# sgartkink/opencl-spmv-algorithms

Measured on AMD Instinct MI355X. Metric: effective HBM GB/s + GFLOP/s per format on cant.mtx, 1/2/4/8 MI355X, higher is better.
Workload: dtype f64

## Files before the change

### include/spmv_ext.h

```cpp
#ifndef SPMV_EXT_H
#define SPMV_EXT_H

#include "spmv.h"

#ifdef __cplusplus
extern "C" {
#endif

size_t spmv_coo_tail_bytes(int64_t nnz);
int spmv_coo_tail_build(spmv_dims d, const int32_t *row, void *tails, size_t tails_bytes);
int spmv_coo_run_tail(spmv_dims d, const int32_t *row, const int32_t *col, const double *val,
                      const double *x, double *y, const void *tails);

int spmv_csr_run_variant(spmv_dims d, const int64_t *row_ptr,
                         const int32_t *col, const double *val,
                         const double *x, double *y, int lanes_per_row,
                         int variant);
size_t spmv_csr_xwin_bytes(int64_t n_rows, int64_t nnz, int lanes_per_row, int32_t rows_per_window);
int spmv_csr_xwin_build(spmv_dims d, const int64_t *row_ptr, const int32_t *col, int lanes_per_row,
                        int32_t rows_per_window, void *win, size_t win_bytes, int32_t *xcap);
int spmv_csr_run_xwin(spmv_dims d, const int64_t *row_ptr, const int32_t *col, const double *val,
                      const double *x, double *y, int lanes_per_row, int32_t rows_per_window,
                      const void *win, int32_t xcap);
int spmv_csr16_run(spmv_dims d, const int64_t *row_ptr, const int32_t *blk_base,
// ... 132 lines not shown

int spmv_dev_csr_from_coo(spmv_dims d, const int32_t *row, const int32_t *col, const double *val,
                          int64_t *row_ptr, int32_t *col_out, double *val_out);
int spmv_dev_ell_plan(spmv_dims d, const int64_t *row_ptr, int32_t ki, int32_t *K, int64_t *ld);
int spmv_dev_ell_fill(spmv_dims d, const int64_t *row_ptr, const int32_t *col, const double *val,
                      int32_t K, int64_t ld, int32_t ki, int32_t *col_out, double *val_out);
int spmv_dev_sell_plan(spmv_dims d, const int64_t *row_ptr, const int32_t *col, int32_t C,
                       int32_t sigma, int32_t ki, int64_t n_slices, int32_t *perm, int64_t *slice_ptr,
                       int32_t *slice_col, int64_t *stored);
int spmv_dev_sell_fill(spmv_dims d, const int64_t *row_ptr, const int32_t *col, const double *val,
                       int32_t C, int32_t ki, int64_t n_slices, const int64_t *slice_ptr,
                       const int32_t *perm, const int32_t *slice_col, int32_t *col_out,
                       double *val_out);
int spmv_dev_cmrs_build(spmv_dims d, const int64_t *row_ptr, int32_t h, int64_t *strip_ptr,
                        uint8_t *row_in_strip);
int spmv_dev_csr_transpose(spmv_dims d, const int64_t *row_ptr, const int32_t *col, const double *val,
                           int64_t *t_ptr, int32_t *t_col, double *t_val);

size_t spmv_dot_ws_bytes(int64_t n);
int spmv_dot(int64_t n, const double *a, const double *b, double *out, void *ws,
             size_t ws_bytes, int device, void *stream);
int spmv_axpy_ratio(int64_t n, const double *num, const double *den, double sign,
                    const double *x, double *y, int device, void *stream);
int spmv_xpay_ratio(int64_t n, const double *num, const double *den, const double *x,
                    double *y, int device, void *stream);
int spmv_scale_rsqrt(int64_t n, const double *s, const double *x, double *y, int device,
                     void *stream);
int spmv_gather(int64_t n, const int32_t *order, const double *x, double *out, int device, void *stream);

enum spmv_option {
    SPMV_OPT_XWIN_REMAP = 1,
    SPMV_OPT_XCD_REMAP = 2,
    SPMV_OPT_STREAM_NT = 3,
    SPMV_OPT_CSR_PREFETCH = 4
};
int spmv_set_option(int option, int value);
int spmv_get_option(int option);


#ifdef __cplusplus
}
#endif

#endif
```

### opencl-spmv-algorithms_amd/csrc/common.h

```cpp
#pragma once

#include <hip/hip_runtime.h>
#include <stdint.h>

#include <type_traits>

#include "spmv.h"
#include "spmv_ext.h"

namespace spmv {

constexpr int kWave = 64;
constexpr int kBlock = 256;

int fail(int rc, const char *where, hipError_t e);
int fail_msg(int rc, const char *msg);

template <int V0, int... Vs, typename F>
inline auto with_int(int v, F &&f)
{
    if constexpr (sizeof...(Vs) == 0)
        return f(std::integral_constant<int, V0>{});
    else if (v == V0)
        return f(std::integral_constant<int, V0>{});
    else
        return with_int<Vs...>(v, f);
}

template <typename F>
inline auto with_bool(bool b, F &&f)
{
    if (b)
        return f(std::true_type{});
    else
        return f(std::false_type{});
}

class DeviceGuard {
  public:
    explicit DeviceGuard(int dev);
    ~DeviceGuard();
    int rc() const { return rc_; }

  private:
    int prev_ = -1;
    int rc_ = SPMV_SUCCESS;
};

bool xcd_remap_enabled();
bool xwin_remap(bool dflt);
bool csr_prefetch(bool dflt);
bool sell_small(int32_t C, int64_t n_slices);

int launch_cmrs_staged(const spmv_dims &d, int32_t h, int64_t n_strips,
                       const int64_t *strip_ptr, const uint8_t *rin, const int32_t *col,
                       const double *val, const double *x, double *y, const int2 *win = nullptr,
                       int32_t xcap = 0);
void cmrs_geometry(const spmv_dims &d, int32_t h, int64_t n_strips, int *L, int *G, int64_t *blocks);
int launch_coo_staged(const spmv_dims &d, const int32_t *row, const int32_t *col,
                      const double *val, const double *x, double *y, int32_t *carry_row,
                      double *carry_val, const int2 *win = nullptr, int32_t xcap = 0,
                      const int32_t *tails = nullptr);
int64_t coo_tail_build(const spmv_dims &d, const int32_t *row, int32_t *tails);
int64_t coo_tail_cap();
int windows_download(const void *win, int64_t n, hipStream_t st, int2 **host, const char *who);
int windows_xcap(const void *win, int64_t n, int32_t cap, hipStream_t st, int32_t *xcap, const char *who);
constexpr int32_t kStagedXwinCap = 2048;
int64_t coo_staged_tile();
int64_t coo_hot_tile(int64_t n_rows, int64_t nnz);
int launch_coo_staged_acc(const spmv_dims &d, const int32_t *row, const int32_t *col,
                          const double *val, const double *x, double *y, int32_t *carry_row,
                          double *carry_val, const int32_t *tails = nullptr);
int launch_csr_tiled(const spmv_dims &d, const int64_t *row_ptr, const int32_t *col,
                     const double *val, const double *x, double *y, int32_t *own_lo,
                     int32_t *carry_row, double *carry_val);
int64_t csr_tiled_tile(int64_t n_rows, int64_t nnz);
int64_t csr_tiled_tile_min();
template <typename V>
int launch_csr_tiled_hot(const spmv_dims &d, const int64_t *row_ptr, const int32_t *col,
                         const V *val, const double *x, double *y, int64_t H, const int32_t *hot,
                         double *xh, const int32_t *own_lo_plan, int32_t *own_lo, int32_t *carry_row,
                         double *carry_val, const int32_t *big = nullptr, int64_t big_len = 0);
int launch_cmrs_tiled(const spmv_dims &d, int32_t h, int64_t n_strips, const int64_t *strip_ptr,
                      const uint8_t *rin, const int32_t *col, const double *val, const double *x,
                      double *y, int32_t *own_lo, int32_t *carry_row, double *carry_val, int64_t H = 0,
                      const int32_t *hot = nullptr, double *xh = nullptr, bool own_lo_ready = false);
int cmrs_tiled_planned(const spmv_dims &d, int32_t h, int64_t n_strips, const int64_t *strip_ptr,
                       const uint8_t *rin, const int32_t *col, const double *val, const double *x, double *y,
                       int64_t H, const int32_t *hot, void *ws, bool fill);
__global__ void csr_tile_rows_kernel(int64_t n_rows, int64_t nnz, int64_t tiles, int64_t ch,
                                     const int64_t *__restrict__ ptr, int32_t *__restrict__ own_lo);
struct XHot;
int launch_coo_staged_acc_hot(const spmv_dims &d, const int32_t *row, const int32_t *col,
                              const double *val, const double *x, double *y, int32_t *carry_row,
                              double *carry_val, const XHot xs);
int launch_coo_staged_hot(const spmv_dims &d, const int32_t *row, const int32_t *col, const double *val,
                          const double *x, double *y, int32_t *carry_row, double *carry_val, int64_t H,
                          const int32_t *hot, double *xh);
int64_t cmrs_tiled_tile(int64_t n_rows, int64_t nnz);
// ... 244 lines not shown
```

### opencl-spmv-algorithms_amd/csrc/csr.hip

```cpp
#include <stdio.h>
#include <stdlib.h>

#include <type_traits>

#include "common.h"

namespace spmv {

template <int L, typename XS>
__device__ __forceinline__ double row_dot_pairs(int64_t beg, int64_t end, int lane,
                                                const int32_t *__restrict__ col,
                                                const double *__restrict__ val, const XS &xs)
{
    double s0 = 0.0, s1 = 0.0, s2 = 0.0, s3 = 0.0;
    int64_t p = (beg & ~(int64_t)1) + 2 * lane;
    for (; p + 1 + 2 * L < end; p += 4 * L) {
        const double2 va = *reinterpret_cast<const double2 *>(val + p);
        const int2 ca = *reinterpret_cast<const int2 *>(col + p);
        const double2 vb = *reinterpret_cast<const double2 *>(val + p + 2 * L);
        const int2 cb = *reinterpret_cast<const int2 *>(col + p + 2 * L);
        s0 += (p >= beg ? va.x : 0.0) * xs(ca.x);
        s1 += va.y * xs(ca.y);
        s2 += vb.x * xs(cb.x);
        s3 += vb.y * xs(cb.y);
// ... 14 lines not shown
template <int L>
__global__ __launch_bounds__(kBlock) void csr_vector_kernel(
    int64_t n_rows, const int64_t *__restrict__ row_ptr,
    const int32_t *__restrict__ col, const double *__restrict__ val,
    const double *__restrict__ x, double *__restrict__ y, int remap)
{
    constexpr int RPB = kBlock / L;
    __shared__ int64_t s_ptr[RPB + 1];

    const int64_t row0 = xcd_block(remap) * RPB;
    if (threadIdx.x <= RPB) {
        int64_t r = row0 + threadIdx.x;
        s_ptr[threadIdx.x] = row_ptr[r < n_rows ? r : n_rows];
    }
    __syncthreads();

    const int g = threadIdx.x / L;
    const int lane = threadIdx.x % L;
    const int64_t row = row0 + g;
    const int64_t beg = s_ptr[g], end = s_ptr[g + 1];
    const double sum = row_dot_pairs<L>(beg, end, lane, col, val, XGlobal{x});
    if (lane == 0 && row < n_rows)
        store_y(y + (row), sum);
}

constexpr int kStageRoundsDefault = 3;
constexpr int64_t kChunkAlign = 32;
__host__ __device__ __forceinline__ int64_t chunk_start(int64_t e) { return e & ~(kChunkAlign - 1); }
constexpr bool kCsrStreamNtDefault = false;
constexpr bool kCsrXwinNtDefault = true;

template <bool NT>
struct Col32 {
    const int32_t *__restrict__ col;
    using Raw = int2;
    __device__ __forceinline__ int2 pair(int64_t p) const { return stream_load2<NT>(col + p); }
    __device__ __forceinline__ int32_t one(int64_t p) const { return stream_load<NT>(col + p); }
    __device__ __forceinline__ Raw raw(int64_t p) const { return stream_load2<NT>(col + p); }
    __device__ __forceinline__ int2 decode(Raw r, int64_t) const { return r; }
};

template <bool NT>
struct Col16 {
    const int32_t *__restrict__ base;
    const uint16_t *__restrict__ off;
    const int32_t *__restrict__ esc;
    __device__ __forceinline__ int2 pair(int64_t p) const
    {
        const int32_t b = base[p >> 6];
        if (b >= 0) {
            const uint32_t w = stream_load<NT>(reinterpret_cast<const uint32_t *>(off + p));
            return int2{b + (int32_t)(w & 0xffffu), b + (int32_t)(w >> 16)};
        }
        return stream_load2<NT>(esc + (int64_t)(-1 - b) * 64 + (p & 63));
    }
    __device__ __forceinline__ int32_t one(int64_t p) const
    {
        const int32_t b = base[p >> 6];
        return b >= 0 ? b + (int32_t)stream_load<NT>(off + p) : esc[(int64_t)(-1 - b) * 64 + (p & 63)];
    }
    struct Raw {
        int32_t b;
        uint32_t w;
    };
    __device__ __forceinline__ Raw raw(int64_t p) const
    {
        return Raw{base[p >> 6], stream_load<NT>(reinterpret_cast<const uint32_t *>(off + p))};
    }
    __device__ __forceinline__ int2 decode(Raw r, int64_t p) const
    {
        if (r.b >= 0)
            return int2{r.b + (int32_t)(r.w & 0xffffu), r.b + (int32_t)(r.w >> 16)};
        return stream_load2<NT>(esc + (int64_t)(-1 - r.b) * 64 + (p & 63));
    }
};

template <int L, int R, bool NT, typename Cols = Col32<NT>, typename XS = XGlobal, typename V = double>
__device__ __forceinline__ void staged_group(
    int64_t row, const int64_t *s_ptr, double2 *s_prod,
    const Cols cols, const V *__restrict__ val,
    const XS xs, double *__restrict__ y, int64_t n_rows)
{
    constexpr int RPB = kBlock / L;
    constexpr int CH = 2 * kBlock * R;
    const int g = threadIdx.x / L;
    const int lane = threadIdx.x % L;
    const int64_t beg = s_ptr[g], end = s_ptr[g + 1];
    const int64_t blk_end = s_ptr[RPB];
    const double *prod = reinterpret_cast<const double *>(s_prod);

    double acc = 0.0;
    for (int64_t cb = chunk_start(s_ptr[0]); cb < blk_end; cb += CH) {
        const int64_t ce = cb + CH < blk_end ? cb + CH : blk_end;
#pragma unroll
        for (int k = 0; k < R; ++k) {
            const int t = threadIdx.x + k * kBlock;
            const int64_t p = cb + 2 * (int64_t)t;
            double2 pr = {0.0, 0.0};
            if (p + 1 < ce) {
                const double2 v = vpair<NT>(val + p);
                const int2 c = cols.pair(p);
                pr.x = v.x * xs(c.x);
                pr.y = v.y * xs(c.y);
            } else if (p < ce) {
                pr.x = vone<NT>(val + p) * xs(cols.one(p));
            }
// ... 172 lines not shown
    }
    for (; grp < n_groups; grp += gridDim.x) {
        if (threadIdx.x <= RPB)
            s_ptr[threadIdx.x] = next;
        __syncthreads();
        const int64_t g2 = grp + gridDim.x;
        if (threadIdx.x <= RPB && g2 < n_groups) {
            int64_t r = g2 * RPB + threadIdx.x;
            next = row_ptr[r < n_rows ? r : n_rows];
        }
        staged_group<L, R, NT, Cols>(grp * RPB + threadIdx.x / L, s_ptr, s_prod, cols, val, XGlobal{x}, y, n_rows);
    }
}

__global__ __launch_bounds__(kBlock) void csr_window_kernel(int64_t n_rows, int64_t rpb,
                                                            const int64_t *__restrict__ row_ptr,
                                                            const int32_t *__restrict__ col,
                                                            int2 *__restrict__ win)
{
    const int64_t g = blockIdx.x;
    const int64_t r1 = (g + 1) * rpb < n_rows ? (g + 1) * rpb : n_rows;
    const int64_t nz = row_ptr[n_rows];
    const int64_t b = row_ptr[g * rpb], e = row_ptr[r1];
    int2 r = {0, -1};
    if (b < e) {
        const int64_t lo = chunk_start(b) >= 2 ? chunk_start(b) - 2 : 0;
        const int64_t hi = e + 1 < nz ? e + 1 : nz;
        r = block_col_range(col, lo, hi);
    }
    if (threadIdx.x == 0)
        win[g] = r;
}

template <int L, int R, bool NT, typename V, int MODE, typename Cols>
__global__ __launch_bounds__(kBlock) void csr_xwin_kernel(
    int64_t n_rows, int64_t n_groups, int64_t gpw, const int64_t *__restrict__ row_ptr,
    const Cols cols, const V *__restrict__ val,
    const double *__restrict__ x, double *__restrict__ y, const int2 *__restrict__ win, int32_t xcap,
    int remap)
{
    static_assert(MODE == 0 || MODE == 3 || MODE == 4, "csr_xwin_kernel: MODE 0, 3 or 4");
    CSR_STAMP(0);
    constexpr int RPB = kBlock / L;
    extern __shared__ double s_x[];
    __shared__ int64_t s_ptr[MODE >= 3 ? 1 : RPB + 1];
    __shared__ double2 s_prod[kBlock * R];
    int64_t *s_off = reinterpret_cast<int64_t *>(s_x + xcap);
    const int64_t nz = row_ptr[n_rows];
    const int64_t wi = xcd_block(remap);
    const int64_t g_beg = wi * gpw;
    const int64_t g_end = (wi + 1) * gpw < n_groups ? (wi + 1) * gpw : n_groups;
    int64_t pb = 0, pe = 0, b0 = 0;
    if constexpr (MODE == 4) {
        const int64_t r0p = g_beg * RPB;
        const int64_t r1 = r0p + RPB < n_rows ? r0p + RPB : n_rows;
        b0 = row_ptr[r0p];
        pe = row_ptr[r1];
    }
    const int2 wnd = win[wi];
    if constexpr (MODE == 4) {
        asm volatile("" ::"s"(b0), "s"(pe), "s"(wnd.x), "s"(wnd.y), "s"(nz));
        pb = chunk_start(b0);
    }
    const int32_t span = wnd.y - wnd.x + 1;
    const bool staged = span > 0 && span <= xcap;
    if constexpr (MODE >= 3) {
// ... 26 lines not shown
                const int32_t i = (int32_t)threadIdx.x + k * kBlock;
                if (i < nr)
                    s_off[i] = o[k];
            }
            if (staged) {
#pragma unroll
                for (int k = 0; k < XU; ++k) {
                    const int32_t i = (int32_t)threadIdx.x + k * kBlock;
                    if (i < span)
                        s_x[i] = xv[k];
                }
            }
        } else {
        pre = false;
        for (int32_t b = 0; b < nr; b += U * kBlock) {
            int64_t o[U];
#pragma unroll
            for (int k = 0; k < U; ++k) {
                const int64_t r = r0 + b + threadIdx.x + k * kBlock;
                o[k] = row_ptr[r < n_rows ? r : n_rows];
            }
            if (staged && b == 0)
                copy_window(s_x, x, wnd.x, span);
#pragma unroll
            for (int k = 0; k < U; ++k) {
                const int32_t i = b + (int32_t)threadIdx.x + k * kBlock;
                if (i < nr)
                    s_off[i] = o[k];
            }
        }
        }
        __syncthreads();
        CSR_STAMP(1);
        if (staged)
            staged_window_pipelined<L, R, NT, XWindow, V, Cols>(r0, (int)(g_end - g_beg), s_off, s_prod, cols, val,
                                                               XWindow{s_x, wnd.x}, y, n_rows, nz, st, pre);
        else
            staged_window_pipelined<L, R, NT, XGlobal, V, Cols>(r0, (int)(g_end - g_beg), s_off, s_prod, cols, val,
                                                               XGlobal{x}, y, n_rows, nz, st, pre);
        return;
    }
    if (staged)
        for (int32_t i = threadIdx.x; i < span; i += kBlock)
            s_x[i] = x[wnd.x + i];
    for (int64_t grp = g_beg; grp < g_end; ++grp) {
        if (threadIdx.x <= RPB) {
            const int64_t r = grp * RPB + threadIdx.x;
            s_ptr[threadIdx.x] = row_ptr[r < n_rows ? r : n_rows];
        }
        __syncthreads();
        const int64_t row = grp * RPB + threadIdx.x / L;
        if (staged)
            staged_group<L, R, NT, Cols, XWindow, V>(row, s_ptr, s_prod, cols, val, XWindow{s_x, wnd.x}, y, n_rows);
        else
            staged_group<L, R, NT, Cols, XGlobal, V>(row, s_ptr, s_prod, cols, val, XGlobal{x}, y, n_rows);
    }
}

static int csr_stage_rounds(int64_t n_rows, int64_t nnz, int L)
{
    if (n_rows <= 0 || L <= 0)
        return kStageRoundsDefault;
    const double eg = (double)(kBlock / L) * ((double)nnz / (double)n_rows);
    const int64_t c3 = (int64_t)((eg + 1535.0) / 1536.0), c4 = (int64_t)((eg + 2047.0) / 2048.0);
    return c4 < c3 ? 4 : 3;
}

static int cu_count()
{
    int dev = 0, n = 0;
    if (hipGetDevice(&dev) != hipSuccess ||
        hipDeviceGetAttribute(&n, hipDeviceAttributeMultiprocessorCount, dev) != hipSuccess || n <= 0)
        n = 256;
    return n;
}

template <typename K>
static int64_t persistent_grid(K kernel, int64_t groups, size_t dyn_lds = 0)
{
    int per_cu = 0;
    if (hipOccupancyMaxActiveBlocksPerMultiprocessor(&per_cu, kernel, kBlock, dyn_lds) != hipSuccess ||
        per_cu <= 0)
        per_cu = 1;
    if (per_cu > 8)
        per_cu = 8;
// ... 158 lines not shown
static void launch_csr_xwin(const spmv_dims &d, const int64_t *row_ptr, const Cols cols,
                            const V *val, const double *x, double *y, const int2 *win, int32_t xcap,
                            int64_t gpw)
{
    constexpr int RPB = kBlock / L;
    const int64_t groups = (d.n_rows + RPB - 1) / RPB;
    const int64_t n_win = (groups + gpw - 1) / gpw;
    int mode = csr_xwin_mode(d.n_rows, d.nnz, gpw * RPB, R);
    if (mode == 3 && csr_xwin_lds(mode, xcap, gpw, RPB) + sizeof(double2) * kBlock * R * 2 > 64 * 1024)
        mode = 0;
    const size_t lds = csr_xwin_lds(mode, xcap, gpw, RPB);
    const int remap = csr_xwin_remap_rule(xcap, gpw * RPB, n_win) ? 1 : 0;
    const hipStream_t st = (hipStream_t)d.stream;
    if (mode == 3 && d.nnz >= 2 && csr_xwin_prefetch_rule(n_win))
        mode = 4;
    with_int<4, 3, 0>(mode, [&](auto M) {
        hipLaunchKernelGGL((csr_xwin_kernel<L, R, NT, V, decltype(M)::value, Cols>), dim3((unsigned)n_win),
                           dim3(kBlock), lds, st, d.n_rows, groups, gpw, row_ptr, cols, val, x, y, win, xcap, remap);
    });
}

struct MakeCol32 {
    const int32_t *col;
    template <bool NT>
    Col32<NT> get() const { return Col32<NT>{col}; }
};

struct MakeCol16 {
    const int32_t *base;
    const uint16_t *off;
    const int32_t *esc;
    template <bool NT>
    Col16<NT> get() const { return Col16<NT>{base, off, esc}; }
};

template <typename V, typename MakeCols>
static int launch_xwin_any(const spmv_dims &d, int L, const int64_t *row_ptr, MakeCols mk, const V *val,
                           const double *x, double *y, const int2 *w, int32_t xcap, int64_t gpw)
{
    if (!lanes_ok(L))
        return fail_msg(SPMV_OTHER_ERROR, "csr x-window run: lanes_per_row must be 0 or a power of two in [2,64]");
    const bool nt = stream_nt(kCsrXwinNtDefault);
    with_int<2, 4, 8, 16, 32, 64>(L, [&](auto Lc) {
        with_int<4, 3>(csr_stage_rounds(d.n_rows, d.nnz, decltype(Lc)::value), [&](auto Rc) {
            with_bool(nt, [&](auto NT) {
                launch_csr_xwin<decltype(Lc)::value, decltype(Rc)::value, decltype(NT)::value>(
                    d, row_ptr, mk.template get<decltype(NT)::value>(), val, x, y, w, xcap, gpw);
            });
        });
    });
    return SPMV_SUCCESS;
}

}

extern "C" size_t spmv_csr_xwin_bytes(int64_t n_rows, int64_t nnz, int lanes_per_row, int32_t rows_per_window)
{
    const int L = lanes_per_row > 0 ? lanes_per_row : spmv_csr_auto_lanes(n_rows, nnz);
    if (L < 2 || L > 64 || (L & (L - 1)) || n_rows <= 0 || rows_per_window < 0)
        return 0;
    const int64_t rpw = csr_xwin_gpw(L, rows_per_window, n_rows) * (kBlock / L);
    return (size_t)((n_rows + rpw - 1) / rpw) * sizeof(int2);
}

extern "C" int spmv_csr_xwin_build(spmv_dims d, const int64_t *row_ptr, const int32_t *col,
                                   int lanes_per_row, int32_t rows_per_window, void *win, size_t win_bytes,
// ... 30 lines not shown
    }
    if (d.n_rows > 0 && (!win || xcap < 0 || xcap > kCsrXwinCap)) {
        snprintf(msg, sizeof msg, "%s: bad window arguments", who);
        return fail_msg(SPMV_OTHER_ERROR, msg);
    }
    *L = lanes_per_row > 0 ? lanes_per_row : spmv_csr_auto_lanes(d.n_rows, d.nnz);
    if (!lanes_ok(*L)) {
        snprintf(msg, sizeof msg, "%s: lanes_per_row must be 0 or a power of two in [2,64]", who);
        return fail_msg(SPMV_OTHER_ERROR, msg);
    }
    *gpw = csr_xwin_gpw(*L, rows_per_window, d.n_rows);
    const int64_t groups = (d.n_rows + kBlock / *L - 1) / (kBlock / *L);
    if ((groups + *gpw - 1) / *gpw > INT32_MAX) {
        snprintf(msg, sizeof msg, "%s: grid too large", who);
        return fail_msg(SPMV_OTHER_ERROR, msg);
    }
    return SPMV_SUCCESS;
}

extern "C" int spmv_csr_run_xwin(spmv_dims d, const int64_t *row_ptr, const int32_t *col, const double *val,
                                 const double *x, double *y, int lanes_per_row, int32_t rows_per_window,
                                 const void *win, int32_t xcap)
{
    int L = 0;
    int64_t gpw = 0;
    int rc = xwin_args(d, rows_per_window, win, xcap, lanes_per_row, &L, &gpw, "spmv_csr_run_xwin");
    if (rc != SPMV_SUCCESS || d.n_rows == 0)
        return rc;
    SPMV_GUARD(d);
    rc = launch_xwin_any(d, L, row_ptr, MakeCol32{col}, val, x, y, (const int2 *)win, xcap, gpw);
    if (rc != SPMV_SUCCESS)
        return rc;
    SPMV_CHECK_LAUNCH("csr_xwin_kernel");
    return SPMV_SUCCESS;
}

extern "C" int spmv_csr16_run(spmv_dims d, const int64_t *row_ptr, const int32_t *blk_base,
                              const uint16_t *col_off, const int32_t *col_esc, const double *val,
                              const double *x, double *y, int lanes_per_row)
{
    if (d.n_rows < 0 || d.n_cols < 0 || d.nnz < 0)
        return fail_msg(SPMV_OTHER_ERROR, "spmv_csr16_run: negative size");
    if (d.n_rows == 0)
        return SPMV_SUCCESS;
    if (d.nnz > 0 && (!blk_base || !col_off))
        return fail_msg(SPMV_OTHER_ERROR, "spmv_csr16_run: missing index arrays");
    SPMV_GUARD(d);
    const int L = lanes_per_row > 0 ? lanes_per_row : spmv_csr_auto_lanes(d.n_rows, d.nnz);
    const bool nt = stream_nt(kCsrStreamNtDefault);
    if (!lanes_ok(L))
        return fail_msg(SPMV_OTHER_ERROR,
                        "spmv_csr16_run: lanes_per_row must be 0 or a power of two in [2,64]");
    with_int<2, 4, 8, 16, 32, 64>(L, [&](auto Lc) {
        with_bool(nt, [&](auto NT) {
            launch_csr16<decltype(Lc)::value, decltype(NT)::value>(
                d, row_ptr, Col16<decltype(NT)::value>{blk_base, col_off, col_esc}, val, x, y);
        });
    });
    SPMV_CHECK_LAUNCH("csr16 kernel");
    return SPMV_SUCCESS;
}

extern "C" int spmv_csr16_run_xwin(spmv_dims d, const int64_t *row_ptr, const int32_t *blk_base,
                                   const uint16_t *col_off, const int32_t *col_esc, const double *val,
                                   const double *x, double *y, int lanes_per_row, int32_t rows_per_window,
                                   const void *win, int32_t xcap)
// ... 237 lines not shown
```

### opencl-spmv-algorithms_amd/csrc/plan.h

```cpp
#pragma once

#include "common.h"

struct spmv_plan {
    int fmt;
    int path;
    spmv_dims d;
    spmv_plan_opts o;
    const int64_t *ptr = nullptr;
    const int32_t *row = nullptr, *col = nullptr, *perm = nullptr;
    const uint8_t *rin = nullptr;
    const double *val = nullptr;
    int32_t K = 0, C = 0, sigma = 0, ki = 0, h = 0, lanes = 0, variant = 0, xwin_rows = 0;
    int64_t ld = 0, n_slices = 0, n_strips = 0;
    void *win = nullptr;
    int32_t xcap = 0;
    void *head = nullptr;
    size_t head_bytes = 0;
    void *tails = nullptr;
    void *ws = nullptr;
    size_t ws_bytes = 0;
    int32_t *own_lo = nullptr;
    int32_t *big = nullptr;
    int64_t big_len = 0, big_tiles = 0, big_tile = 0;
    int32_t split_T = 0;
    bool tiles_planned = false;
    int64_t n_chunks = 0;
    int32_t *chunk_slice = nullptr, *chunk_k0 = nullptr;
    uint16_t *col16 = nullptr;
    int32_t *hcol = nullptr;
    int32_t *hot = nullptr;
    int64_t H = 0;
    size_t owned = 0;
    char kernel[64] = "";
    char desc[320] = "";
    int32_t t_mode = 0;
    int32_t t_xcap = 0;
    int64_t t_blocks = 0, t_lds_blocks = 0, t_flush = 0;
    int32_t t_mxcap[4] = {0, 0, 0, 0};
    int64_t t_mlds[4] = {0, 0, 0, 0};
    void *t_win = nullptr;
    int64_t *t_ptr = nullptr;
    int32_t *t_col = nullptr;
    double *t_val = nullptr;
    spmv_plan *t_inner = nullptr;
    size_t t_owned = 0;
    int32_t m_mode = 0;
    spmv_multi_opts m_req = {-1, -1};
    int32_t m_seg_len = 0;
    int64_t m_long_entries = 0;
    spmv::MultiBalance m_bal;
    size_t m_owned = 0;
};

namespace spmv {
void plan_multi_free(spmv_plan *p);
void plan_transpose_free(spmv_plan *p);
}
```

### opencl-spmv-algorithms_amd/csrc/plan.hip

```cpp
#include <stdio.h>
#include <stdlib.h>
#include <string.h>

#include <new>

#include "common.h"
#include "plan.h"
#include "spmv_host.h"

namespace spmv {

enum PlanPath {
    P_COO_CARRY,
    P_COO_TAIL,
    P_COO_XWIN,
    P_COO_HOT,
    P_CSR_VARIANT,
    P_CSR_XWIN,
    P_CSR_TILED,
    P_ELL,
    P_ELL_XWIN,
    P_SELL,
    P_SELL_XWIN,
    P_SELL_XWIN_HEAD,
    P_SELL_SPLIT,
    P_SELL_HOT,
    P_SELL16,
    P_CMRS,
    P_CMRS_XWIN,
    P_CMRS_TILED,
};

__global__ __launch_bounds__(kBlock) void max_len_kernel(int64_t n, const int64_t *__restrict__ off,
                                                         int64_t *__restrict__ out)
{
    __shared__ int64_t s_m[kBlock / kWave];
    int64_t m = 0;
    for (int64_t i = (int64_t)blockIdx.x * kBlock + threadIdx.x; i < n; i += (int64_t)gridDim.x * kBlock) {
        const int64_t l = off[i + 1] - off[i];
        m = l > m ? l : m;
    }
#pragma unroll
    for (int o = kWave / 2; o > 0; o >>= 1) {
        const int64_t t = __shfl_xor(m, o);
        m = t > m ? t : m;
    }
    if ((threadIdx.x & (kWave - 1)) == 0)
        s_m[threadIdx.x / kWave] = m;
    __syncthreads();
    if (threadIdx.x == 0) {
        for (int w = 1; w < kBlock / kWave; ++w)
            m = s_m[w] > m ? s_m[w] : m;
        out[blockIdx.x] = m;
    }
}

static void multi_tables_free(MultiBalance &m)
{
    for (const void *q : {(const void *)m.seg_beg, (const void *)m.seg_cnt, (const void *)m.seg_dest,
                          (const void *)m.long_row, (const void *)m.long_first, (const void *)m.part})
        if (q)
            (void)hipFree(const_cast<void *>(q));
    m = MultiBalance();
}
// ... 148 lines not shown
int check_dims(const spmv_dims &d, const char *who)
{
    static thread_local char msg[128];
    if (d.n_rows < 0 || d.n_cols < 0 || d.nnz < 0) {
        snprintf(msg, sizeof msg, "%s: negative sizes", who);
        return fail_msg(SPMV_OTHER_ERROR, msg);
    }
    return SPMV_SUCCESS;
}

}

extern "C" {

void spmv_plan_opts_init(spmv_plan_opts *o)
{
    if (!o)
        return;
    memset(o, 0, sizeof *o);
    o->variant = -1;
    o->xwin = -1;
    o->head = -1;
    o->coo_pass = -1;
    o->split = -1;
    o->bigplan = -1;
    o->H = -1;
}

int spmv_plan_destroy(spmv_plan *p)
{
    if (!p)
        return SPMV_SUCCESS;
    void *owned[] = {p->win,    p->head,        p->tails,    p->ws,    p->own_lo, p->big,
                     p->chunk_slice, p->chunk_k0, p->col16, p->hcol, p->hot};
    int dev = -1;
    (void)hipGetDevice(&dev);
    if (dev != p->d.device)
        (void)hipSetDevice(p->d.device);
    plan_transpose_free(p);
    plan_multi_free(p);
    for (void *q : owned)
        if (q)
            (void)hipFree(q);
    if (dev >= 0 && dev != p->d.device)
        (void)hipSetDevice(dev);
    delete p;
    return SPMV_SUCCESS;
}

int spmv_plan_coo(spmv_dims d, const int32_t *row, const int32_t *col, const double *val, const spmv_plan_opts *o,
                  spmv_plan **out)
{
    if (!out)
        return fail_msg(SPMV_OTHER_ERROR, "spmv_plan_coo: out is NULL");
    *out = nullptr;
    int rc = check_dims(d, "spmv_plan_coo");
    if (rc != SPMV_SUCCESS)
        return rc;
    if (d.nnz > 0 && (!row || !col || !val))
        return fail_msg(SPMV_OTHER_ERROR, "spmv_plan_coo: NULL array");
    spmv_plan *p = new_plan(SPMV_FMT_COO, d, o);
    if (!p)
        return fail_msg(SPMV_OTHER_ERROR, "spmv_plan_coo: out of host memory");
    SPMV_GUARD(d);
    p->row = row;
    p->col = col;
    p->val = val;
// ... 98 lines not shown
                const int64_t nb = spmv_csr_tiled_bigplan(d.n_rows, hp, p->big_tile, 1024, nullptr);
                if (nb > tiles) {
                    int32_t *bp = (int32_t *)malloc((size_t)nb * sizeof(int32_t));
                    if (!bp) {
                        free(hp);
                        return finish(p, fail_msg(SPMV_OTHER_ERROR, "spmv_plan_csr: out of host memory"), out);
                    }
                    spmv_csr_tiled_bigplan(d.n_rows, hp, p->big_tile, 1024, bp);
                    for (int64_t t = 0; t < tiles; ++t)
                        p->big_tiles += bp[t] >= 0;
                    if (p->big_tiles > 0) {
                        rc = plan_upload(p, (void **)&p->big, bp, (size_t)nb * sizeof(int32_t));
                        p->big_len = nb;
                    }
                    free(bp);
                }
                free(hp);
                if (rc != SPMV_SUCCESS)
                    return finish(p, rc, out);
            }
        }
        snprintf(p->kernel, sizeof p->kernel, "csr_tiled_kernel");
        snprintf(p->desc, sizeof p->desc,
                 "CSR: entry-balanced tiles of %lld entries (skewed rows), tile plan, %lld big tiles listed%s",
                 (long long)p->big_tile, (long long)p->big_tiles, H > 0 ? ", hot-column table" : "");
        return finish(p, rc, out);
    }
    if (xwin_on(p->o, true) && (v == 0 || v == 3)) {
        p->path = P_CSR_XWIN;
        p->variant = 3;
        const size_t wb = spmv_csr_xwin_bytes(d.n_rows, d.nnz, p->lanes, p->xwin_rows);
        if ((rc = plan_alloc(p, &p->win, wb)) == SPMV_SUCCESS)
            rc = spmv_csr_xwin_build(d, row_ptr, col, p->lanes, p->xwin_rows, p->win, wb, &p->xcap);
        snprintf(p->kernel, sizeof p->kernel, "csr_xwin_kernel");
        snprintf(p->desc, sizeof p->desc, "CSR-vector: %d lanes per row, x windows of %d rows in LDS (xcap %d)",
                 p->lanes, p->xwin_rows > 0 ? p->xwin_rows : 128, p->xcap);
        return finish(p, rc, out);
    }
    p->path = P_CSR_VARIANT;
    static const char *names[] = {"csr_staged_persistent_kernel", "csr_vector_kernel", "csr_staged_kernel",
                                  "csr_staged_persistent_kernel"};
    snprintf(p->kernel, sizeof p->kernel, "%s", names[v]);
    snprintf(p->desc, sizeof p->desc, "CSR-vector: %d lanes per row, variant %d, global x gathers", p->lanes,
             v == 0 ? 3 : v);
    return finish(p, SPMV_SUCCESS, out);
}

int spmv_plan_ell(spmv_dims d, int32_t K, int64_t ld, int32_t ki, const int32_t *col, const double *val,
                  const spmv_plan_opts *o, spmv_plan **out)
{
    if (!out)
        return fail_msg(SPMV_OTHER_ERROR, "spmv_plan_ell: out is NULL");
    *out = nullptr;
    int rc = check_dims(d, "spmv_plan_ell");
    if (rc != SPMV_SUCCESS)
        return rc;
    if (K < 0 || ld < d.n_rows || ld % kWave != 0 || (ki != 1 && ki != 2) || K % ki != 0 ||
        (K > 0 && (!col || !val)))
        return fail_msg(SPMV_OTHER_ERROR, "spmv_plan_ell: bad ELL geometry (K, ld, ki) or NULL array");
    spmv_plan *p = new_plan(SPMV_FMT_ELL, d, o);
    if (!p)
        return fail_msg(SPMV_OTHER_ERROR, "spmv_plan_ell: out of host memory");
    SPMV_GUARD(d);
    p->K = K;
    p->ld = ld;
    p->ki = ki;
    p->col = col;
    p->val = val;
    if (xwin_on(p->o, true)) {
// ... 216 lines not shown
        const size_t wb = spmv_cmrs_xwin_bytes(d, h, n_strips);
        if ((rc = plan_alloc(p, &p->win, wb)) == SPMV_SUCCESS)
            rc = spmv_cmrs_xwin_build(d, h, n_strips, strip_ptr, col, p->win, wb, &p->xcap);
        snprintf(p->desc, sizeof p->desc, "CMRS h=%d: staged strip runs, x windows in LDS (xcap %d)", h, p->xcap);
        return finish(p, rc, out);
    }
    p->path = P_CMRS;
    snprintf(p->desc, sizeof p->desc, "CMRS h=%d: staged strip runs, global x gathers", h);
    return finish(p, SPMV_SUCCESS, out);
}

int spmv_plan_run(const spmv_plan *p, const double *x, double *y, void *stream)
{
    if (!p)
        return fail_msg(SPMV_OTHER_ERROR, "spmv_plan_run: plan is NULL");
    if ((p->d.n_rows > 0 && !y) || (p->d.nnz > 0 && p->d.n_cols > 0 && !x))
        return fail_msg(SPMV_OTHER_ERROR, "spmv_plan_run: x or y is NULL");
    spmv_dims d = p->d;
    d.stream = stream;
    const int64_t H = p->H;
    const int32_t *col = run_col(p);
    switch (p->path) {
    case P_COO_CARRY:
        return spmv_coo_run(d, p->row, p->col, p->val, x, y, p->ws, p->ws_bytes);
    case P_COO_TAIL:
        return spmv_coo_run_tail(d, p->row, p->col, p->val, x, y, p->tails);
    case P_COO_XWIN:
        return spmv_coo_run_xwin(d, p->row, p->col, p->val, x, y, p->ws, p->ws_bytes, p->win, p->xcap);
    case P_COO_HOT:
        return spmv_coo_run_hot(d, p->row, col, p->val, x, y, H, p->hot, p->ws, p->ws_bytes);
    case P_CSR_VARIANT:
        return spmv_csr_run_variant(d, p->ptr, p->col, p->val, x, y, p->lanes, p->variant);
    case P_CSR_XWIN:
        return spmv_csr_run_xwin(d, p->ptr, p->col, p->val, x, y, p->lanes, p->xwin_rows, p->win, p->xcap);
    case P_CSR_TILED:
        if (p->big)
            return spmv_csr_run_tiled_plan(d, p->ptr, col, p->val, x, y, H, p->hot, p->own_lo, p->big,
                                           p->big_len, p->big_tile, p->ws, p->ws_bytes);
        return spmv_csr_run_tiled_hot(d, p->ptr, col, p->val, x, y, H, p->hot, p->own_lo, p->ws, p->ws_bytes);
    case P_ELL:
        return spmv_ell_run(d, p->K, p->ld, p->ki, p->col, p->val, x, y);
    case P_ELL_XWIN:
        return spmv_ell_run_xwin(d, p->K, p->ld, p->ki, p->col, p->val, x, y, p->win, p->xcap);
    case P_SELL:
        return spmv_sell_run(d, p->C, p->sigma, p->ki, p->n_slices, p->ptr, p->perm, p->col, p->val, x, y);
    case P_SELL_XWIN:
        return spmv_sell_run_xwin(d, p->C, p->sigma, p->ki, p->n_slices, p->ptr, p->perm, p->col, p->val, x, y,
                                  p->win, p->xcap);
    case P_SELL_XWIN_HEAD:
        return spmv_sell_run_xwin_head(d, p->C, p->sigma, p->ki, p->n_slices, p->ptr, p->perm, p->col, p->val, x, y,
                                       p->win, p->xcap, p->head);
    case P_SELL_SPLIT:
        return spmv_sell_run_split(d, p->C, p->sigma, p->ki, p->n_slices, p->ptr, p->perm, p->col, p->val, x, y,
                                   p->win, p->xcap, p->split_T, p->n_chunks, p->chunk_slice, p->chunk_k0, p->ws,
                                   p->ws_bytes);
    case P_SELL_HOT:
        return spmv_sell_run_hot(d, p->C, p->sigma, p->ki, p->n_slices, p->ptr, p->perm, col, p->val, x, y,
                                 p->split_T > 0 ? p->split_T : INT32_MAX, p->split_T > 0 ? p->n_chunks : 0,
                                 p->chunk_slice, p->chunk_k0, H, p->hot, p->ws, p->ws_bytes);
    case P_SELL16:
        return spmv_sell16_run(d, p->C, p->sigma, p->ki, p->n_slices, p->ptr, p->perm, p->col16, p->val, x, y, p->win,
                               p->xcap, p->head);
    case P_CMRS:
        return spmv_cmrs_run(d, p->h, p->n_strips, p->ptr, p->rin, p->col, p->val, x, y);
    case P_CMRS_XWIN:
        return spmv_cmrs_run_xwin(d, p->h, p->n_strips, p->ptr, p->rin, p->col, p->val, x, y, p->win, p->xcap);
// ... 194 lines not shown
    info->mode = p->m_mode;
    if (p->m_mode == SPMV_M_NONE)
        return SPMV_SUCCESS;
    info->long_len = p->m_bal.long_len;
    info->seg_len = p->m_seg_len;
    info->long_rows = p->m_bal.n_long;
    info->segments = p->m_bal.n_seg;
    info->slots = p->m_bal.n_slots;
    info->long_entries = p->m_long_entries;
    info->owned_bytes = (int64_t)p->m_owned;
    if (p->t_inner) {
        info->t_long_rows = p->t_inner->m_bal.n_long;
        info->t_segments = p->t_inner->m_bal.n_seg;
        info->t_owned_bytes = (int64_t)p->t_inner->m_owned;
    }
    snprintf(info->kernel, sizeof info->kernel, "%s", p->m_bal.n_seg > 0 ? "csr_multi_long_kernel" : "csr_multi_kernel");
    return SPMV_SUCCESS;
}

int spmv_plan_get_info(const spmv_plan *p, spmv_plan_info *info)
{
    if (!p || !info)
        return fail_msg(SPMV_OTHER_ERROR, "spmv_plan_get_info: NULL argument");
    memset(info, 0, sizeof *info);
    info->format = p->fmt;
    info->path = p->path;
    info->lanes = p->lanes;
    info->variant = p->variant;
    info->ki = p->ki;
    info->xcap = p->xcap;
    info->xwin = p->win != nullptr;
    info->head = p->head != nullptr;
    info->single_pass = p->path == P_COO_TAIL;
    info->index16 = p->path == P_SELL16;
    info->split_T = p->split_T;
    info->n_chunks = p->n_chunks;
    info->big_tiles = p->big_tiles;
    info->head_bytes = (int64_t)p->head_bytes;
    info->ws_bytes = (int64_t)p->ws_bytes;
    info->owned_bytes = (int64_t)p->owned;
    info->H = p->H;
    snprintf(info->kernel, sizeof info->kernel, "%s", p->kernel);
    snprintf(info->desc, sizeof info->desc, "%s", p->desc);
    return SPMV_SUCCESS;
}

}
```

### opencl-spmv-algorithms_amd/csrc/runtime.hip

```cpp
#include <stdio.h>
#include <stdlib.h>
#include <string.h>

#include <atomic>

#include "common.h"

namespace spmv {

static thread_local char g_last_error[512] = "";

int fail(int rc, const char *where, hipError_t e)
{
    snprintf(g_last_error, sizeof g_last_error, "%s: %s (%d)", where,
             hipGetErrorString(e), (int)e);
    return rc;
}

int fail_msg(int rc, const char *msg)
{
    snprintf(g_last_error, sizeof g_last_error, "%s", msg);
    return rc;
}

DeviceGuard::DeviceGuard(int dev)
{
    hipError_t e = hipGetDevice(&prev_);
    if (e != hipSuccess) {
        rc_ = fail(SPMV_DEVICE_ERROR, "hipGetDevice", e);
        prev_ = -1;
        return;
    }
    if (prev_ != dev) {
        e = hipSetDevice(dev);
        if (e != hipSuccess)
            rc_ = fail(SPMV_DEVICE_ERROR, "hipSetDevice", e);
    }
}

DeviceGuard::~DeviceGuard()
{
    int cur = -1;
    if (prev_ >= 0 && hipGetDevice(&cur) == hipSuccess && cur != prev_)
        (void)hipSetDevice(prev_);
}

static int env_switch(const char *name)
{
    const char *s = getenv(name);
    return (s && (s[0] == '0' || s[0] == '1') && s[1] == 0) ? s[0] - '0' : -1;
}
static std::atomic<int> g_opt_xwin_remap{env_switch("SPMV_XWIN_REMAP")};
static std::atomic<int> g_opt_xcd_remap{env_switch("SPMV_XCD_REMAP")};
static std::atomic<int> g_opt_stream_nt{env_switch("SPMV_STREAM_NT")};
static std::atomic<int> g_opt_csr_prefetch{env_switch("SPMV_CSR_PREFETCH")};

static std::atomic<int> *option_slot(int option)
{
    switch (option) {
    case SPMV_OPT_XWIN_REMAP:
        return &g_opt_xwin_remap;
    case SPMV_OPT_XCD_REMAP:
        return &g_opt_xcd_remap;
    case SPMV_OPT_STREAM_NT:
        return &g_opt_stream_nt;
    case SPMV_OPT_CSR_PREFETCH:
        return &g_opt_csr_prefetch;
    default:
        return nullptr;
    }
}

bool xwin_remap(bool dflt)
{
    const int v = g_opt_xwin_remap.load(std::memory_order_relaxed);
    return v < 0 ? dflt : v == 1;
}

bool xcd_remap_enabled() { return g_opt_xcd_remap.load(std::memory_order_relaxed) == 1; }

bool csr_prefetch(bool dflt)
{
    const int v = g_opt_csr_prefetch.load(std::memory_order_relaxed);
    return v < 0 ? dflt : v == 1;
}

bool stream_nt(bool dflt)
{
    const int v = g_opt_stream_nt.load(std::memory_order_relaxed);
    return v < 0 ? dflt : v == 1;
}

static void *g_flush[64];
static size_t g_flush_bytes[64];

__global__ __launch_bounds__(kBlock) void flush_read_kernel(const uint4 *__restrict__ p, int64_t n16,
                                                            uint32_t *__restrict__ sink)
{
    uint32_t acc = 0;
    for (int64_t i = (int64_t)blockIdx.x * kBlock + threadIdx.x; i < n16; i += (int64_t)gridDim.x * kBlock) {
        const uint4 v = p[i];
        acc ^= v.x ^ v.y ^ v.z ^ v.w;
    }
    if (acc == 0x9e3779b9u && sink)
        sink[threadIdx.x] = acc;
}

static int flush_scratch(size_t bytes, void **buf)
{
    int dev = 0;
    hipError_t e = hipGetDevice(&dev);
    if (e != hipSuccess)
        return fail(SPMV_DEVICE_ERROR, "hipGetDevice", e);
    if (dev < 0 || dev >= 64)
        return fail_msg(SPMV_DEVICE_ERROR, "device ordinal out of range");
    if (g_flush_bytes[dev] < bytes) {
// ... 266 lines not shown
```

### opencl-spmv-algorithms_amd/spmv_amd.py

```python
from __future__ import annotations

import ctypes
import os
import sys
from dataclasses import dataclass, field
from pathlib import Path

import numpy as np

PKG_DIR = Path(__file__).resolve().parent
LIB_DIR = PKG_DIR / "lib"
REPO_DIR = PKG_DIR.parent

FORMATS = ("coo", "csr", "ell", "sell", "cmrs")
EXTRA_FORMATS = ("csr16", "hyb", "csrf32", "sell16", "csrg")
ALL_FORMATS = FORMATS + EXTRA_FORMATS
HBM_PEAK_GBS = 8000.0

SUCCESS, DEVICE_ERROR, PROGRAM_ERROR, FILE_ERROR, OTHER_ERROR = range(5)


class SpmvError(RuntimeError):

    def __init__(self, rc: int, what: str, detail: str = ""):
# ... 960 lines not shown
        return {"mode": {v: k for k, v in TRANSPOSE_MODES.items()}[info.mode],
                "cap_cols": [int(v) for v in info.cap_cols], "lds_blocks": [int(v) for v in info.lds_blocks],
                "kernel": info.kernel.decode()}

    def run_t_multi(self, X, Y, stream=None) -> None:
        torch = _torch()
        for t in (X, Y):
            if not isinstance(t, torch.Tensor) or t.dtype != torch.float64:
                raise SpmvError(OTHER_ERROR, "run_t_multi", "X and Y must be float64 tensors")
            if t.dim() != 2:
                raise SpmvError(OTHER_ERROR, "run_t_multi", "X and Y must be 2-D (rows, k)")
        k = X.shape[1]
        if k < 1 or Y.shape[1] != k:
            raise SpmvError(OTHER_ERROR, "run_t_multi", "X and Y must have the same number k >= 1 of columns")
        if X.shape[0] < self.n_rows or Y.shape[0] < self.n_cols:
            raise SpmvError(OTHER_ERROR, "run_t_multi", "X or Y has too few rows")
        for t in (X, Y):
            if (k > 1 and t.stride(1) != 1) or (t.shape[0] > 1 and t.stride(0) < k):
                raise SpmvError(OTHER_ERROR, "run_t_multi", "X and Y need inner stride 1 and a row stride >= k")
        here = torch.device(self.device)
        idx = here.index or 0
        for t in (X, Y):
            if t.device.type != here.type or (t.device.index or 0) != idx:
                raise SpmvError(OTHER_ERROR, "run_t_multi", f"X and Y must be on {here.type}:{idx}")
        if self.plan is None:
            raise SpmvError(OTHER_ERROR, "run_t_multi", f"format {self.fmt} has no plan: no transposed run")
        ldx = X.stride(0) if X.shape[0] > 1 else k
        ldy = Y.stride(0) if Y.shape[0] > 1 else k
        st = stream if stream is not None else torch.cuda.current_stream(here)
        _check(hip_lib().spmv_plan_run_t_multi(self.plan, k, _ptr(X), ldx, _ptr(Y), ldy, st.cuda_stream),
               f"spmv_plan_run_t_multi ({self.fmt})")


OPTIONS = {"xwin_remap": 1, "xcd_remap": 2, "stream_nt": 3, "csr_prefetch": 4}


def set_option(name: str, value: int | None) -> None:
    _check(hip_lib().spmv_set_option(OPTIONS[name], -1 if value is None else int(value)), f"set_option {name}")


def get_option(name: str) -> int:
    return int(hip_lib().spmv_get_option(OPTIONS[name]))


def _tri(v) -> int:
    return -1 if v is None else int(bool(v))


def plan_opts(**kw) -> PlanOpts:
    o = PlanOpts()
    hip_lib().spmv_plan_opts_init(ctypes.byref(o))
    for k, v in kw.items():
        setattr(o, k, v)
    return o


_PLAN_INFO_KEYS = ("lanes", "variant", "ki", "xcap", "xwin", "head", "single_pass", "index16", "split_T", "n_chunks",
                   "big_tiles", "head_bytes", "ws_bytes", "owned_bytes", "H")


def _attach_plan(dm: DeviceMatrix, what: str, create, *args, opts: PlanOpts) -> None:
    plan = _vp()
    _check(create(dm.dims(), *args, ctypes.byref(opts), ctypes.byref(plan)), what)
    dm.plan = plan
    info = PlanInfo()
    _check(hip_lib().spmv_plan_get_info(plan, ctypes.byref(info)), "spmv_plan_get_info")
    for k in _PLAN_INFO_KEYS:
# ... 344 lines not shown
```

Baseline: 3969.

## Store CSR column indices as 16-bit window-relative offsets in x-window plans

Result: faster. 4462, median of 6 (+12.4%).

```diff
diff --git a/include/spmv_ext.h b/include/spmv_ext.h
--- a/include/spmv_ext.h
+++ b/include/spmv_ext.h
@@ -188,7 +188,8 @@
     SPMV_OPT_XWIN_REMAP = 1,
     SPMV_OPT_XCD_REMAP = 2,
     SPMV_OPT_STREAM_NT = 3,
-    SPMV_OPT_CSR_PREFETCH = 4
+    SPMV_OPT_CSR_PREFETCH = 4,
+    SPMV_OPT_CSR_COL16 = 5
 };
 int spmv_set_option(int option, int value);
 int spmv_get_option(int option);
diff --git a/opencl-spmv-algorithms_amd/csrc/common.h b/opencl-spmv-algorithms_amd/csrc/common.h
--- a/opencl-spmv-algorithms_amd/csrc/common.h
+++ b/opencl-spmv-algorithms_amd/csrc/common.h
@@ -50,6 +50,7 @@
 bool xcd_remap_enabled();
 bool xwin_remap(bool dflt);
 bool csr_prefetch(bool dflt);
+bool csr_col16(bool dflt);
 bool sell_small(int32_t C, int64_t n_slices);
 
 int launch_cmrs_staged(const spmv_dims &d, int32_t h, int64_t n_strips,
@@ -65,6 +66,14 @@
 int64_t coo_tail_cap();
 int windows_download(const void *win, int64_t n, hipStream_t st, int2 **host, const char *who);
 int windows_xcap(const void *win, int64_t n, int32_t cap, hipStream_t st, int32_t *xcap, const char *who);
+size_t csr_col16_bytes(int64_t nnz);
+int csr_col16_fits(const spmv_dims &d, int lanes_per_row, int32_t rows_per_window, const void *win, int32_t xcap,
+                   bool *fits);
+int csr_col16_fill(const spmv_dims &d, const int64_t *row_ptr, const int32_t *col, int lanes_per_row,
+                   int32_t rows_per_window, const void *win, uint16_t *off);
+int csr_run_xwin_col16(spmv_dims d, const int64_t *row_ptr, const uint16_t *off, const double *val,
+                       const double *x, double *y, int lanes_per_row, int32_t rows_per_window, const void *win,
+                       int32_t xcap);
 constexpr int32_t kStagedXwinCap = 2048;
 int64_t coo_staged_tile();
 int64_t coo_hot_tile(int64_t n_rows, int64_t nnz);
diff --git a/opencl-spmv-algorithms_amd/csrc/csr.hip b/opencl-spmv-algorithms_amd/csrc/csr.hip
--- a/opencl-spmv-algorithms_amd/csrc/csr.hip
+++ b/opencl-spmv-algorithms_amd/csrc/csr.hip
@@ -70,6 +70,7 @@
 
 template <bool NT>
 struct Col32 {
+    static constexpr bool kWindowRelative = false;
     const int32_t *__restrict__ col;
     using Raw = int2;
     __device__ __forceinline__ int2 pair(int64_t p) const { return stream_load2<NT>(col + p); }
@@ -80,6 +81,7 @@
 
 template <bool NT>
 struct Col16 {
+    static constexpr bool kWindowRelative = false;
     const int32_t *__restrict__ base;
     const uint16_t *__restrict__ off;
     const int32_t *__restrict__ esc;
@@ -110,6 +112,33 @@
         if (r.b >= 0)
             return int2{r.b + (int32_t)(r.w & 0xffffu), r.b + (int32_t)(r.w >> 16)};
         return stream_load2<NT>(esc + (int64_t)(-1 - r.b) * 64 + (p & 63));
+    }
+};
+
+template <bool NT>
+struct ColWin16 {
+    static constexpr bool kWindowRelative = true;
+    const uint16_t *__restrict__ off;
+    using Raw = uint32_t;
+    __device__ __forceinline__ Raw raw(int64_t p) const
+    {
+        return stream_load<NT>(reinterpret_cast<const uint32_t *>(off + p));
+    }
+    __device__ __forceinline__ int2 decode(Raw w, int64_t) const
+    {
+        return int2{(int32_t)(w & 0xffffu), (int32_t)(w >> 16)};
+    }
+    __device__ __forceinline__ int2 pair(int64_t p) const { return decode(raw(p), p); }
+    __device__ __forceinline__ int32_t one(int64_t p) const { return (int32_t)stream_load<NT>(off + p); }
+};
+
+struct XWindowRel {
+    const double *s;
+    uint32_t hi;
+    __device__ __forceinline__ double operator()(int32_t o) const
+    {
+        const uint32_t u = (uint32_t)o;
+        return s[u < hi ? u : hi];
     }
 };
 
@@ -348,6 +377,23 @@
         win[g] = r;
 }
 
+__global__ __launch_bounds__(kBlock) void csr_col16_kernel(int64_t n_rows, int64_t nnz, int64_t rpb,
+                                                           const int64_t *__restrict__ row_ptr,
+                                                           const int32_t *__restrict__ col,
+                                                           const int2 *__restrict__ win,
+                                                           uint16_t *__restrict__ off)
+{
+    const int64_t g = blockIdx.x;
+    const int64_t r1 = (g + 1) * rpb < n_rows ? (g + 1) * rpb : n_rows;
+    const int64_t b = row_ptr[g * rpb];
+    const int64_t e = row_ptr[r1] < nnz ? row_ptr[r1] : nnz;
+    const int32_t lo = win[g].x;
+    for (int64_t p = b + threadIdx.x; p < e; p += kBlock)
+        off[p] = (uint16_t)(col[p] - lo);
+    if (g == 0 && threadIdx.x < 2)
+        off[nnz + threadIdx.x] = 0;
+}
+
 template <int L, int R, bool NT, typename V, int MODE, typename Cols>
 __global__ __launch_bounds__(kBlock) void csr_xwin_kernel(
     int64_t n_rows, int64_t n_groups, int64_t gpw, const int64_t *__restrict__ row_ptr,
@@ -440,7 +486,11 @@
         }
         __syncthreads();
         CSR_STAMP(1);
-        if (staged)
+        if constexpr (Cols::kWindowRelative)
+            staged_window_pipelined<L, R, NT, XWindowRel, V, Cols>(r0, (int)(g_end - g_beg), s_off, s_prod, cols,
+                                                                  val, XWindowRel{s_x, staged ? (uint32_t)span - 1 : 0u},
+                                                                  y, n_rows, nz, st, pre);
+        else if (staged)
             staged_window_pipelined<L, R, NT, XWindow, V, Cols>(r0, (int)(g_end - g_beg), s_off, s_prod, cols, val,
                                                                XWindow{s_x, wnd.x}, y, n_rows, nz, st, pre);
         else
@@ -458,7 +508,10 @@
         }
         __syncthreads();
         const int64_t row = grp * RPB + threadIdx.x / L;
-        if (staged)
+        if constexpr (Cols::kWindowRelative)
+            staged_group<L, R, NT, Cols, XWindowRel, V>(row, s_ptr, s_prod, cols, val,
+                                                        XWindowRel{s_x, staged ? (uint32_t)span - 1 : 0u}, y, n_rows);
+        else if (staged)
             staged_group<L, R, NT, Cols, XWindow, V>(row, s_ptr, s_prod, cols, val, XWindow{s_x, wnd.x}, y, n_rows);
         else
             staged_group<L, R, NT, Cols, XGlobal, V>(row, s_ptr, s_prod, cols, val, XGlobal{x}, y, n_rows);
@@ -683,6 +736,12 @@
     const int32_t *esc;
     template <bool NT>
     Col16<NT> get() const { return Col16<NT>{base, off, esc}; }
+};
+
+struct MakeColWin16 {
+    const uint16_t *off;
+    template <bool NT>
+    ColWin16<NT> get() const { return ColWin16<NT>{off}; }
 };
 
 template <typename V, typename MakeCols>
@@ -779,6 +838,65 @@
     if (rc != SPMV_SUCCESS)
         return rc;
     SPMV_CHECK_LAUNCH("csr_xwin_kernel");
+    return SPMV_SUCCESS;
+}
+
+size_t spmv::csr_col16_bytes(int64_t nnz)
+{
+    return ((size_t)2 * (size_t)(nnz + 2) + 3) & ~(size_t)3;
+}
+
+int spmv::csr_col16_fits(const spmv_dims &d, int lanes_per_row, int32_t rows_per_window, const void *win,
+                         int32_t xcap, bool *fits)
+{
+    *fits = false;
+    const int64_t n_win = (int64_t)(spmv_csr_xwin_bytes(d.n_rows, d.nnz, lanes_per_row, rows_per_window) / sizeof(int2));
+    if (d.nnz < 2 || n_win <= 0 || !win || xcap < 1 || xcap > kCsrXwinCap)
+        return SPMV_SUCCESS;
+    int2 *h = nullptr;
+    const int rc = windows_download(win, n_win, (hipStream_t)d.stream, &h, "spmv_plan_csr");
+    if (rc != SPMV_SUCCESS)
+        return rc;
+    bool ok = true;
+    for (int64_t w = 0; w < n_win && ok; ++w) {
+        const int64_t span = (int64_t)h[w].y - h[w].x + 1;
+        ok = span == 0 || (span > 0 && span <= xcap);
+    }
+    free(h);
+    *fits = ok;
+    return SPMV_SUCCESS;
+}
+
+int spmv::csr_col16_fill(const spmv_dims &d, const int64_t *row_ptr, const int32_t *col, int lanes_per_row,
+                         int32_t rows_per_window, const void *win, uint16_t *off)
+{
+    const int L = lanes_per_row > 0 ? lanes_per_row : spmv_csr_auto_lanes(d.n_rows, d.nnz);
+    if (!lanes_ok(L) || d.n_rows <= 0 || !win || !off)
+        return fail_msg(SPMV_OTHER_ERROR, "spmv_plan_csr: 16-bit column copy: bad arguments");
+    const int64_t rpw = csr_xwin_gpw(L, rows_per_window, d.n_rows) * (kBlock / L);
+    const int64_t n_win = (d.n_rows + rpw - 1) / rpw;
+    hipLaunchKernelGGL(csr_col16_kernel, dim3((unsigned)n_win), dim3(kBlock), 0, (hipStream_t)d.stream, d.n_rows,
+                       d.nnz, rpw, row_ptr, col, (const int2 *)win, off);
+    SPMV_CHECK_LAUNCH("csr_col16_kernel");
+    return SPMV_SUCCESS;
+}
+
+int spmv::csr_run_xwin_col16(spmv_dims d, const int64_t *row_ptr, const uint16_t *off, const double *val,
+                             const double *x, double *y, int lanes_per_row, int32_t rows_per_window,
+                             const void *win, int32_t xcap)
+{
+    int L = 0;
+    int64_t gpw = 0;
+    int rc = xwin_args(d, rows_per_window, win, xcap, lanes_per_row, &L, &gpw, "spmv_plan_run");
+    if (rc != SPMV_SUCCESS || d.n_rows == 0)
+        return rc;
+    if (!off || xcap < 1 || d.nnz < 2)
+        return fail_msg(SPMV_OTHER_ERROR, "spmv_plan_run: corrupt 16-bit column copy");
+    SPMV_GUARD(d);
+    rc = launch_xwin_any(d, L, row_ptr, MakeColWin16{off}, val, x, y, (const int2 *)win, xcap, gpw);
+    if (rc != SPMV_SUCCESS)
+        return rc;
+    SPMV_CHECK_LAUNCH("csr_xwin_kernel (16-bit window offsets)");
     return SPMV_SUCCESS;
 }
 
diff --git a/opencl-spmv-algorithms_amd/csrc/plan.h b/opencl-spmv-algorithms_amd/csrc/plan.h
--- a/opencl-spmv-algorithms_amd/csrc/plan.h
+++ b/opencl-spmv-algorithms_amd/csrc/plan.h
@@ -28,6 +28,7 @@
     int64_t n_chunks = 0;
     int32_t *chunk_slice = nullptr, *chunk_k0 = nullptr;
     uint16_t *col16 = nullptr;
+    uint16_t *cwin16 = nullptr;
     int32_t *hcol = nullptr;
     int32_t *hot = nullptr;
     int64_t H = 0;
diff --git a/opencl-spmv-algorithms_amd/csrc/plan.hip b/opencl-spmv-algorithms_amd/csrc/plan.hip
--- a/opencl-spmv-algorithms_amd/csrc/plan.hip
+++ b/opencl-spmv-algorithms_amd/csrc/plan.hip
@@ -30,6 +30,8 @@
     P_CMRS_XWIN,
     P_CMRS_TILED,
 };
+
+constexpr bool kCsrCol16Rule = true;
 
 __global__ __launch_bounds__(kBlock) void max_len_kernel(int64_t n, const int64_t *__restrict__ off,
                                                          int64_t *__restrict__ out)
@@ -244,7 +246,7 @@
     if (!p)
         return SPMV_SUCCESS;
     void *owned[] = {p->win,    p->head,        p->tails,    p->ws,    p->own_lo, p->big,
-                     p->chunk_slice, p->chunk_k0, p->col16, p->hcol, p->hot};
+                     p->chunk_slice, p->chunk_k0, p->col16, p->cwin16, p->hcol, p->hot};
     int dev = -1;
     (void)hipGetDevice(&dev);
     if (dev != p->d.device)
@@ -409,9 +411,18 @@
         const size_t wb = spmv_csr_xwin_bytes(d.n_rows, d.nnz, p->lanes, p->xwin_rows);
         if ((rc = plan_alloc(p, &p->win, wb)) == SPMV_SUCCESS)
             rc = spmv_csr_xwin_build(d, row_ptr, col, p->lanes, p->xwin_rows, p->win, wb, &p->xcap);
+        bool c16 = false;
+        if (rc == SPMV_SUCCESS && csr_col16(kCsrCol16Rule))
+            rc = csr_col16_fits(d, p->lanes, p->xwin_rows, p->win, p->xcap, &c16);
+        if (rc == SPMV_SUCCESS && c16 &&
+            (rc = plan_alloc(p, (void **)&p->cwin16, csr_col16_bytes(d.nnz))) == SPMV_SUCCESS &&
+            (rc = csr_col16_fill(d, row_ptr, col, p->lanes, p->xwin_rows, p->win, p->cwin16)) == SPMV_SUCCESS &&
+            hipStreamSynchronize((hipStream_t)d.stream) != hipSuccess)
+            rc = fail_msg(SPMV_PROGRAM_ERROR, "spmv_plan_csr: 16-bit column copy");
         snprintf(p->kernel, sizeof p->kernel, "csr_xwin_kernel");
-        snprintf(p->desc, sizeof p->desc, "CSR-vector: %d lanes per row, x windows of %d rows in LDS (xcap %d)",
-                 p->lanes, p->xwin_rows > 0 ? p->xwin_rows : 128, p->xcap);
+        snprintf(p->desc, sizeof p->desc, "CSR-vector: %d lanes per row, x windows of %d rows in LDS (xcap %d)%s",
+                 p->lanes, p->xwin_rows > 0 ? p->xwin_rows : 128, p->xcap,
+                 p->cwin16 ? ", 16-bit window column offsets (plan-owned)" : "");
         return finish(p, rc, out);
     }
     p->path = P_CSR_VARIANT;
@@ -694,6 +705,8 @@
     case P_CSR_VARIANT:
         return spmv_csr_run_variant(d, p->ptr, p->col, p->val, x, y, p->lanes, p->variant);
     case P_CSR_XWIN:
+        if (p->cwin16)
+            return csr_run_xwin_col16(d, p->ptr, p->cwin16, p->val, x, y, p->lanes, p->xwin_rows, p->win, p->xcap);
         return spmv_csr_run_xwin(d, p->ptr, p->col, p->val, x, y, p->lanes, p->xwin_rows, p->win, p->xcap);
     case P_CSR_TILED:
         if (p->big)
@@ -954,7 +967,7 @@
     info->xwin = p->win != nullptr;
     info->head = p->head != nullptr;
     info->single_pass = p->path == P_COO_TAIL;
-    info->index16 = p->path == P_SELL16;
+    info->index16 = p->path == P_SELL16 || p->cwin16 != nullptr;
     info->split_T = p->split_T;
     info->n_chunks = p->n_chunks;
     info->big_tiles = p->big_tiles;
diff --git a/opencl-spmv-algorithms_amd/csrc/runtime.hip b/opencl-spmv-algorithms_amd/csrc/runtime.hip
--- a/opencl-spmv-algorithms_amd/csrc/runtime.hip
+++ b/opencl-spmv-algorithms_amd/csrc/runtime.hip
@@ -54,6 +54,7 @@
 static std::atomic<int> g_opt_xcd_remap{env_switch("SPMV_XCD_REMAP")};
 static std::atomic<int> g_opt_stream_nt{env_switch("SPMV_STREAM_NT")};
 static std::atomic<int> g_opt_csr_prefetch{env_switch("SPMV_CSR_PREFETCH")};
+static std::atomic<int> g_opt_csr_col16{env_switch("SPMV_CSR_COL16")};
 
 static std::atomic<int> *option_slot(int option)
 {
@@ -66,6 +67,8 @@
         return &g_opt_stream_nt;
     case SPMV_OPT_CSR_PREFETCH:
         return &g_opt_csr_prefetch;
+    case SPMV_OPT_CSR_COL16:
+        return &g_opt_csr_col16;
     default:
         return nullptr;
     }
@@ -82,6 +85,12 @@
 bool csr_prefetch(bool dflt)
 {
     const int v = g_opt_csr_prefetch.load(std::memory_order_relaxed);
+    return v < 0 ? dflt : v == 1;
+}
+
+bool csr_col16(bool dflt)
+{
+    const int v = g_opt_csr_col16.load(std::memory_order_relaxed);
     return v < 0 ? dflt : v == 1;
 }
 
diff --git a/opencl-spmv-algorithms_amd/spmv_amd.py b/opencl-spmv-algorithms_amd/spmv_amd.py
--- a/opencl-spmv-algorithms_amd/spmv_amd.py
+++ b/opencl-spmv-algorithms_amd/spmv_amd.py
@@ -1016,7 +1016,7 @@
                f"spmv_plan_run_t_multi ({self.fmt})")
 
 
-OPTIONS = {"xwin_remap": 1, "xcd_remap": 2, "stream_nt": 3, "csr_prefetch": 4}
+OPTIONS = {"xwin_remap": 1, "xcd_remap": 2, "stream_nt": 3, "csr_prefetch": 4, "csr_col16": 5}
 
 
 def set_option(name: str, value: int | None) -> None:
```
